# samson6460/tf2_YOLO

Measured on AMD Instinct MI355X. Metric: images/sec training YOLOv3 416x416 bs=32/GPU, higher is better.
Workload: dtype f32-storage/fp16x2-mfma

## Files before the change

### include/yolo_hip.h

```cpp
#ifndef YOLO_HIP_H_
#define YOLO_HIP_H_

#include <stddef.h>
#include <stdint.h>

#ifdef __cplusplus
extern "C" {
#endif

typedef enum yolo_status {
  YOLO_OK = 0,
  YOLO_ERR_INVALID_ARG = -1,
  YOLO_ERR_LAUNCH = -2,
  YOLO_ERR_WORKSPACE = -3
} yolo_status;

enum { YOLO_ACT_LINEAR = 0, YOLO_ACT_LEAKY = 1, YOLO_ACT_MISH = 2 };
enum { YOLO_HEAD_V3 = 3, YOLO_HEAD_V2 = 2, YOLO_HEAD_V1 = 1, YOLO_HEAD_V4 = 4 };
enum { YOLO_NMS_HARD = 1, YOLO_NMS_SOFT = 2, YOLO_NMS_DIOU = 3 };

const char* yolo_last_error(void);
int yolo_abi_version(void);
int yolo_device_available(void);
int yolo_mfma_probe(const void* operands_f16, float* sink, int workgroups, int iters, double* flops_host, void* stream);
// ... 9 lines not shown
typedef struct yolo_conv_desc {
  int N, H, W, Cin;
  int Cout, kh, kw;
  int Ho, Wo;
  int sh, sw;
  int pad_t, pad_l;
} yolo_conv_desc;

#define YOLO_BN_STAT_SLOTS 64
#define YOLO_BN_RED_SLOTS 512
#define YOLO_SPLIT_BATCH_UNITS 4

int yolo_conv2d_fwd(const yolo_conv_desc* d, const float* x, const float* w,
                    const float* bias, float* y, double* stats, void* stream);
int yolo_conv2d_fwd_absmax(const yolo_conv_desc* d, const float* x, const float* w, const float* bias,
                           float* y, double* stats, unsigned* absmax, void* stream);

int yolo_conv2d_dgrad(const yolo_conv_desc* d, const float* dy, const float* wT,
                      float* dx, int accumulate, void* stream);

int yolo_conv2d_wgrad(const yolo_conv_desc* d, const float* x, const float* dy,
                      float* dw, float* dbias, void* stream);

int yolo_conv2d_wgrad_bias(const float* dy, long long P, int Cout, float* dbias, void* stream);

int yolo_filter_transpose(const float* w, float* wT, int Cout, int taps, int Cin, void* stream);

size_t yolo_planes_bytes(long long rows, int C);
int yolo_split_planes(const float* x, long long rows, int C, void* planes, void* stream);
int yolo_split_planes_padded(const float* x, long long rows, int C_src, int C, void* planes, void* stream);

int yolo_split_planes_batch(const void* jobs, int njobs, long long total_blocks, void* stream);
int yolo_filter_transpose_batch(const void* jobs, int njobs, long long total_blocks, void* stream);

int yolo_conv2d_fwd_planes(const yolo_conv_desc* d, const void* x_planes, const void* w_planes,
                           const float* bias, float* y, double* stats, unsigned* absmax, void* stream);
int yolo_conv2d_dgrad_planes(const yolo_conv_desc* d, const void* dy_planes, const void* wT_planes,
                             float* dx, int accumulate, void* stream);
enum { YOLO_EPI_NONE = 0, YOLO_EPI_AFFINE = 1, YOLO_EPI_AFFINE_LEAKY = 2, YOLO_EPI_AFFINE_MISH = 3 };
int yolo_conv2d_fwd_planes_epi(const yolo_conv_desc* d, const void* x_planes, const void* w_planes, const float* bias,
                               int epilogue, const float* scale, const float* shift, const float* residual, float* y,
                               unsigned* absmax, void* stream);
int yolo_split_planes_absmax(const float* x, long long rows, int C, const unsigned* absmax, const float* extra_bound,
                             void* planes, float* out_bound, void* stream);
#define YOLO_INFER_BOUND_WORDS 4096
int yolo_conv_pred_bound(const float* w, int Cout, int kdim, const float* scale, const float* shift, const float* bias,
                         float* pred2, void* stream);
int yolo_conv2d_fwd_infer_unit(const yolo_conv_desc* d, const void* x_planes, const void* w_planes, const float* bias,
                               int epilogue, const float* scale, const float* shift, const float* residual, float* y,
                               unsigned* absmax, const float* pred2, const void* in_bound, int in_n,
                               const void* residual_bound, int residual_n, void* out_planes, unsigned* out_words,
                               float* out_bound, int* out_n_host, void* stream);
int yolo_fold_bound(const void* words, int n, float* out_bound, void* stream);
int yolo_absmax_words(const float* x, long long n, unsigned* words, int* n_words_host, void* stream);
int yolo_stem_filter_prep(const float* w, const float* bias, float* wt, void* stream);
int yolo_stem_fwd_infer_unit(const yolo_conv_desc* d, const float* x, const float* wt, int epilogue, const float* scale,
                             const float* shift, const float* pred2, const void* in_bound, int in_n, float* y,
                             void* out_planes, unsigned* out_words, int* out_n_host, void* stream);
int yolo_split_planes_concat(const float* const* srcs_host, const int* channels_host, const float* const* bounds_host,
                             int nsrc, long long rows, void* planes, float* dst32, float* out_bound, void* stream);
int yolo_split_planes_concat_ex(const float* const* srcs_host, const int* channels_host, const float* const* bounds_host,
                                const int* bound_words_host, const int* upsample_host, int H, int W, int nsrc,
                                long long rows, void* planes, float* dst32, float* out_bound, void* stream);
int yolo_conv2d_fwd_head_unit(const yolo_conv_desc* d, const void* x_planes, const void* w_planes, const float* bias,
                              int A, int C, int version, const float* anchors, float* t, float* y, void* stream);
int yolo_conv2d_wgrad_planes(const yolo_conv_desc* d, const void* x_planes, const void* dy_planes,
// ... 189 lines not shown
```

### tf2_yolo_amd/_lib.py

```python
import ctypes
import os
from ctypes import (POINTER, Structure, c_char_p, c_double, c_float, c_int, c_longlong,
                    c_size_t, c_void_p)

from . import tape as _tape

_HERE = os.path.dirname(os.path.abspath(__file__))
LIB_PATH = os.path.join(_HERE, "libyolo_hip.so")

ACT_LINEAR, ACT_LEAKY, ACT_MISH = 0, 1, 2
NMS_HARD, NMS_SOFT, NMS_DIOU = 1, 2, 3


class YoloHipError(RuntimeError):
    pass


class ConvDesc(Structure):
    _fields_ = [(n, c_int) for n in
                ("N", "H", "W", "Cin", "Cout", "kh", "kw", "Ho", "Wo", "sh", "sw", "pad_t", "pad_l")]


class LossCfg(Structure):
    _fields_ = [("version", c_int), ("N", c_int), ("gh", c_int), ("gw", c_int), ("A", c_int),
                ("C", c_int), ("anchors", c_float * 32), ("use_anchors", c_int),
                ("binary_weight", c_float), ("loss_weight", c_float * 4),
                ("ignore_thresh", c_float), ("use_focal_loss", c_int), ("focal_gamma", c_float),
                ("use_scale", c_int), ("wh_reg_weight", c_float), ("truth_thresh", c_float),
                ("label_smooth", c_float)]


_P = c_void_p
_LL = c_longlong
SIGNATURES = {
    "yolo_last_error": (c_char_p, []),
    "yolo_abi_version": (c_int, []),
    "yolo_device_available": (c_int, []),
    "yolo_set_option": (c_int, [c_int, c_int]),
    "yolo_mfma_probe": (c_int, [_P, _P, c_int, c_int, POINTER(c_double), _P]),
    "yolo_set_debug_buffer": (c_int, [_P, c_size_t]),
    "yolo_encode_labels": (c_int, [_P, _P, _P, c_int, c_double, c_double, c_int, c_int, c_int, _P, _P, _P]),
    "yolo_down2xlabel": (c_int, [_P, c_int, c_int, c_int, c_int, _P, _P, _P]),
    "yolo_conv_workspace_bytes": (c_size_t, []),
    "yolo_set_conv_workspace": (c_int, [_P, c_size_t, _P]),
    "yolo_conv2d_fwd": (c_int, [POINTER(ConvDesc), _P, _P, _P, _P, _P, _P]),
    "yolo_conv2d_dgrad": (c_int, [POINTER(ConvDesc), _P, _P, _P, c_int, _P]),
    "yolo_conv2d_wgrad": (c_int, [POINTER(ConvDesc), _P, _P, _P, _P, _P]),
    "yolo_conv2d_wgrad_bias": (c_int, [_P, _LL, c_int, _P, _P]),
    "yolo_filter_transpose": (c_int, [_P, _P, c_int, c_int, c_int, _P]),
    "yolo_planes_bytes": (c_size_t, [_LL, c_int]),
    "yolo_split_planes": (c_int, [_P, _LL, c_int, _P, _P]),
    "yolo_split_planes_padded": (c_int, [_P, _LL, c_int, c_int, _P, _P]),
    "yolo_split_planes_batch": (c_int, [_P, c_int, _LL, _P]),
    "yolo_filter_transpose_batch": (c_int, [_P, c_int, _LL, _P]),
    "yolo_conv2d_fwd_planes": (c_int, [POINTER(ConvDesc), _P, _P, _P, _P, _P, _P, _P]),
    "yolo_stem_bwd_scratch_bytes": (c_size_t, []),
    "yolo_stem_bn_bwd_wgrad": (c_int, [POINTER(ConvDesc), _P, _P, _P, _P, _P, _P, _P, c_int, _P, _P, _P, _P, _P, c_size_t, _P]),
    "yolo_conv2d_fwd_planes_epi": (c_int, [POINTER(ConvDesc), _P, _P, _P, c_int, _P, _P, _P, _P, _P, _P]),
    "yolo_split_planes_absmax": (c_int, [_P, _LL, c_int, _P, _P, _P, _P, _P]),
    "yolo_conv_pred_bound": (c_int, [_P, c_int, c_int, _P, _P, _P, _P, _P]),
    "yolo_conv2d_fwd_infer_unit": (c_int, [POINTER(ConvDesc), _P, _P, _P, c_int, _P, _P, _P, _P, _P, _P, _P, c_int, _P, c_int,
                                           _P, _P, _P, POINTER(c_int), _P]),
    "yolo_fold_bound": (c_int, [_P, c_int, _P, _P]),
    "yolo_absmax_words": (c_int, [_P, _LL, _P, POINTER(c_int), _P]),
    "yolo_stem_filter_prep": (c_int, [_P, _P, _P, _P]),
    "yolo_stem_fwd_infer_unit": (c_int, [POINTER(ConvDesc), _P, _P, c_int, _P, _P, _P, _P, c_int, _P, _P, _P, POINTER(c_int), _P]),
    "yolo_split_planes_concat": (c_int, [POINTER(c_void_p), POINTER(c_int), POINTER(c_void_p), c_int, _LL, _P, _P, _P, _P]),
    "yolo_split_planes_concat_ex": (c_int, [POINTER(c_void_p), POINTER(c_int), POINTER(c_void_p), POINTER(c_int), POINTER(c_int),
                                            c_int, c_int, c_int, _LL, _P, _P, _P, _P]),
    "yolo_conv2d_fwd_head_unit": (c_int, [POINTER(ConvDesc), _P, _P, _P, c_int, c_int, c_int, _P, _P, _P, _P]),
    "yolo_conv2d_fwd_absmax": (c_int, [POINTER(ConvDesc), _P, _P, _P, _P, _P, _P, _P]),
    "yolo_conv2d_dgrad_planes": (c_int, [POINTER(ConvDesc), _P, _P, _P, c_int, _P]),
    "yolo_conv2d_wgrad_planes": (c_int, [POINTER(ConvDesc), _P, _P, _P, _P]),
    "yolo_wgrad_workspace_bytes": (c_size_t, []),
    "yolo_set_wgrad_workspace": (c_int, [_P, c_size_t]),
    "yolo_bn_stats": (c_int, [_P, _LL, c_int, _P, _P]),
    "yolo_bn_finalize": (c_int, [_P, _LL, c_int, _P, _P, c_float, c_float, c_int, _P, _P, _P, _P, _P, _P, _P]),
    "yolo_bn_fold_inference": (c_int, [c_int, _P, _P, _P, _P, c_float, _P, _P, _P]),
    "yolo_bn_act_fwd": (c_int, [_P, _LL, c_int, _P, _P, c_int, _P, _P, _P]),
    "yolo_bn_act_bwd_reduce": (c_int, [_P, _P, _LL, c_int, _P, _P, _P, _P, c_int, _P, _P]),
    "yolo_bn_act_bwd_apply": (c_int, [_P, _P, _LL, c_int, _P, _P, _P, _P, _P, c_int, _P, _P, _P, _P, _P]),
    "yolo_bn_act_fwd_planes": (c_int, [_P, _LL, c_int, _P, _P, c_int, _P, _P, _P, _P, _P, _P, _P]),
    "yolo_bn_act_fwd_res_planes": (c_int, [_P, _LL, c_int, _P, _P, c_int, _P, _P, _P, _P, _P, _P]),
    "yolo_bn_act_bwd_apply_planes": (c_int, [_P, _P, _LL, c_int, _P, _P, _P, _P, _P, c_int, _P, _P, _P, _P, _P, _P,
                                             _P]),
    "yolo_bn_infer_bound": (c_int, [c_int, _P, _P, _P, _P, _P]),
    "yolo_bn_finalize_bound": (c_int, [_P, _LL, c_int, _P, _P, c_float, c_float, c_int, _P, _P, _P, _P, _P, _P, _P,
# ... 116 lines not shown
```

### tf2_yolo_amd/csrc/conv.hip

```cpp
#include "conv_args.hpp"
#include <cstdlib>
#include <type_traits>

namespace yolo {

template <int BM, int BN, int WGM, int WGN, bool FLAT>
__global__ __launch_bounds__(256) void gather_conv_kernel(const GatherConvArgs a) {
  constexpr int BK = 32;
  constexpr int LD = BK + 4;
  constexpr int TM = BM / WGM / 32;
  constexpr int TN = BN / WGN / 32;
  constexpr int AR = BM / 32;
  constexpr int BR = BN / 32;
  static_assert(WGM * WGN == 4, "4 waves per block");
  static_assert(TM >= 1 && TN >= 1, "wave tile");

  extern __shared__ __attribute__((aligned(16))) float smem[];
  constexpr int BUF = (BM + BN) * LD;

  const int tid = threadIdx.x;
  const int lane = tid & 63;
  const int wave = tid >> 6;
  const int wm = wave / WGN, wn = wave % WGN;

// ... 982 lines not shown
  a.dst = t;
  fill_fwd_args(d, a);
  YOLO_REQUIRE(gather_planes_supported(a), "conv_fwd_head_unit: needs Cin %% 16 == 0 and Cout >= 32");
  if ((version == YOLO_HEAD_V3 || version == YOLO_HEAD_V4) && anchors != nullptr) {
    a.head_y = y;
    a.head_anchors = anchors;
    a.head_A = A;
    a.head_C = C;
    if (conv_small_head_supported(a)) {
      int nwg = 0;
      return launch_conv_small(a, as_stream(stream), &nwg);
    }
    a.head_y = nullptr;
  }
  if (int rc = launch_gather_planes(a, as_stream(stream))) return rc;
  return yolo_head_act_fwd(t, (long long)d->N * d->Ho * d->Wo, A, C, version, anchors, y, stream);
}

extern "C" size_t yolo_planes_bytes(long long rows, int C) {
  if (rows <= 0 || C <= 0 || (C % 16) != 0) return 0;
  return (size_t)planes_bytes(rows, C);
}

extern "C" int yolo_split_planes_batch(const void* jobs, int njobs, long long total_blocks, void* stream) {
  YOLO_REQUIRE(jobs, "split_planes_batch: null job table");
  return launch_split_planes_batch(jobs, njobs, total_blocks, as_stream(stream));
}

extern "C" int yolo_filter_transpose_batch(const void* jobs, int njobs, long long total_blocks, void* stream) {
  YOLO_REQUIRE(jobs, "filter_transpose_batch: null job table");
  return launch_filter_transpose_batch(jobs, njobs, total_blocks, as_stream(stream));
}

extern "C" int yolo_split_planes(const float* x, long long rows, int C, void* planes, void* stream) {
  YOLO_REQUIRE(x && planes, "split_planes: null pointer");
  return launch_split_planes(x, rows, C, planes, as_stream(stream));
}

extern "C" int yolo_split_planes_padded(const float* x, long long rows, int C_src, int C, void* planes, void* stream) {
  YOLO_REQUIRE(x && planes, "split_planes_padded: null pointer");
  return launch_split_planes_padded(x, rows, C_src, C, planes, as_stream(stream));
}

struct BnRedArgs {
  const float* y;
  const float* scale;
  const float* shift;
  const float* mean;
  const float* invstd;
  int act;
  float* part;
  int cap;
  unsigned* aux;
  int nslots;
};
static void set_bnred(GatherConvArgs& a, const BnRedArgs* b) {
  if (b == nullptr) return;
  a.bwd_y = b->y; a.bwd_scale = b->scale; a.bwd_shift = b->shift; a.bwd_mean = b->mean; a.bwd_invstd = b->invstd;
  a.bwd_act = b->act; a.bwd_part = b->part; a.bwd_cap = b->cap; a.bwd_aux = b->aux;
}

static int dgrad_impl(const yolo_conv_desc* d, const float* dy, const float* wT, float* dx, int accumulate,
                      void* stream, bool planes, BnRedArgs* bnred = nullptr) {
  if (int rc = validate_desc(d)) return rc;
  YOLO_REQUIRE(dy && wT && dx, "conv_dgrad: null pointer");
  const bool flat = (d->Cout % 32) != 0;
// ... 214 lines not shown
```

### tf2_yolo_amd/csrc/conv_args.hpp

```cpp
#pragma once
#include "common.hpp"

namespace yolo {

constexpr int MAX_TAPS = 49;

struct Tap {
  int oy, ox, woff;
};

struct ClassGeom {
  long long M;
  int Hg, Wg, ooy, oox, tap0, ntaps;
};

struct GatherConvArgs {
  const float* src;
  const float* wgt;
  const float* bias;
  float* dst;
  double* stats;
  unsigned* absmax;
  long long M;
  int N, Hs, Ws, Cs;
// ... 62 lines not shown

struct WgradArgs {
  const float* src;
  const float* dy;
  float* dw;
  long long M;
  int N, Hs, Ws, Cs;
  int Hg, Wg;
  int sy, sx;
  int Cout, ldw;
  int ntaps;
  int kw, pad_t, pad_l;
  int tiles_co, tiles_j;
  int nblocks;
  long long chunk;
  unsigned src_bytes, dy_bytes;
  int zero_blk_src, zero_blk_dy;
  float* slabs;
  int splits;
};

int launch_gather_split(GatherConvArgs& a, hipStream_t st);
bool gather_split_supported(const GatherConvArgs& a);
long long planes_bytes(long long rows, int C);
int launch_split_planes(const float* x, long long rows, int C, void* planes, hipStream_t st);
int launch_split_planes_absmax(const float* x, long long rows, int C, const unsigned* absmax, const float* extra_bound, int extra_n,
                               void* planes, float* out_bound, hipStream_t st);
int launch_split_planes_concat(const float* const* xs, const int* Cs, const float* const* bounds, int nsrc, long long rows,
                               void* planes, float* dst32, float* out_bound, hipStream_t st,
                               const int* bound_words = nullptr, const int* upsample = nullptr, int H = 0, int W = 0);
int launch_split_planes_padded(const float* x, long long rows, int Csrc, int C, void* planes, hipStream_t st);
int launch_split_planes_batch(const void* jobs, int njobs, long long total_blocks, hipStream_t st);
int launch_filter_transpose_batch(const void* jobs, int njobs, long long total_blocks, hipStream_t st);
int launch_gather_planes(GatherConvArgs& a, hipStream_t st);
bool conv_small_supported(const GatherConvArgs& a);
bool conv_small_head_supported(const GatherConvArgs& a);
int launch_conv_small(GatherConvArgs& a, hipStream_t st, int* nwg);
bool gather_planes_supported(const GatherConvArgs& a);
int conv_split_parts(const GatherConvArgs& a, long long nb, int bm, int min_cb, int idle_div);
int launch_split_reduce(GatherConvArgs& a, int bm, hipStream_t st);
float* conv_split_slabs();
int launch_conv_win(GatherConvArgs& a, int variant, hipStream_t st);
bool conv_win_supported(const GatherConvArgs& a);
enum { OPT_CONV_WIN = 0, OPT_STAMPS = 1, OPT_CONV_SK = 2, OPT_DBG = 3, OPT_TILE_ORDER = 4, OPT_CONV_PATCH = 5, OPT_WGRAD_WIN = 6, OPT_NMS_WALK = 7, OPT_EXP = 8, OPT_COUNT = 16 };
int set_conv_workspace(void* p, size_t bytes, hipStream_t st);
extern void* g_dbg_buf;
extern size_t g_dbg_bytes;
extern int g_opt[OPT_COUNT];
void init_options();
int launch_wgrad_planes(WgradArgs& a, hipStream_t st);
bool wgrad_planes_supported(const WgradArgs& a);
int launch_wgrad_win(WgradArgs& a, hipStream_t st);
bool wgrad_win_supported(const WgradArgs& a);
constexpr size_t WGRAD_WS_COLSUM_BYTES = 1 << 20;
void* wgrad_workspace(size_t* bytes);
bool stem_fwd_supported(const yolo_conv_desc* d);
struct StemEpiArgs {
  const float* scale;
  const float* shift;
  int act;
  void* planes;
  const float* pred;
  const unsigned* in_words;
  int in_n;
  unsigned* out_words;
};
// ... 16 lines not shown
```

### tf2_yolo_amd/csrc/conv_planes.hip

```cpp
#include "planes_epilogue.hpp"
#include <algorithm>
#include <cstdlib>
#include <type_traits>

namespace yolo {

__global__ __launch_bounds__(256) void planes_amax_kernel(const float* __restrict__ x, long long n4,
                                                         unsigned* __restrict__ header) {
  float m = 0.f;
  for (long long i = (long long)blockIdx.x * 256 + threadIdx.x; i < n4; i += (long long)gridDim.x * 256) {
    const f32x4 v = reinterpret_cast<const f32x4*>(x)[i];
    m = fmaxf(fmaxf(m, fmaxf(fabsf(v[0]), fabsf(v[1]))), fmaxf(fabsf(v[2]), fabsf(v[3])));
  }
#pragma unroll
  for (int o = 32; o > 0; o >>= 1) m = fmaxf(m, __shfl_xor(m, o, 64));
  __shared__ float wmax[4];
  if ((threadIdx.x & 63) == 0) wmax[threadIdx.x >> 6] = m;
  __syncthreads();
  if (threadIdx.x == 0) {
    m = fmaxf(fmaxf(wmax[0], wmax[1]), fmaxf(wmax[2], wmax[3]));
    if (__builtin_bit_cast(unsigned, m) > *reinterpret_cast<volatile unsigned*>(header))
      atomicMax(header, __builtin_bit_cast(unsigned, m));
  }
}
// ... 603 lines not shown
                               void* planes, float* dst32, float* out_bound, hipStream_t st, const int* bound_words,
                               const int* upsample, int H, int W) {
  ConcatSrcs cs{};
  int C = 0;
  cs.H = H;
  cs.W = W;
  for (int i = 0; i < nsrc; ++i) {
    cs.x[i] = xs[i];
    cs.bound[i] = bounds[i];
    cs.bound_n[i] = bound_words != nullptr ? bound_words[i] : 1;
    cs.up[i] = upsample != nullptr ? upsample[i] : 0;
    cs.C[i] = Cs[i];
    C += Cs[i];
    cs.g_end[i] = C >> 3;
  }
  cs.n = nsrc;
  const long long rows_padded = ((rows + 15) / 16 + 1) * 16;
  const int G = C >> 3;
  const long long blocks = ((rows_padded + 16 * SPLIT_BLOCKS_PER_WG - 1) / (16 * SPLIT_BLOCKS_PER_WG)) * ((G + 15) >> 4);
  if (blocks <= 0 || blocks > 0x7fffffffLL) {
    set_error("split_planes_concat: bad grid %lld", blocks);
    return YOLO_ERR_INVALID_ARG;
  }
  hipLaunchKernelGGL(split_planes_concat_kernel, dim3((unsigned)blocks), dim3(256), 0, st, cs, rows, C,
                     reinterpret_cast<unsigned char*>(planes), rows_padded, dst32, out_bound);
  return check_launch("split_planes_concat_kernel");
}

struct BatchJob {
  const void* src;
  void* dst;
  long long a, b, c, first_block;
};
__device__ __forceinline__ int find_job(const BatchJob* jobs, int njobs, long long block) {
  int lo = 0, hi = njobs - 1;
  while (lo < hi) {
    const int mid = (lo + hi + 1) >> 1;
    if (jobs[mid].first_block <= block) lo = mid;
    else hi = mid - 1;
  }
  return lo;
}

__global__ void planes_header_clear_batch_kernel(const BatchJob* __restrict__ jobs, int njobs) {
  const int i = blockIdx.x * blockDim.x + threadIdx.x;
  if (i >= njobs) return;
  unsigned* header = reinterpret_cast<unsigned*>(reinterpret_cast<unsigned char*>(jobs[i].dst) +
                                                 planes_body_bytes(jobs[i].a, (int)jobs[i].b));
  header[0] = 0u;
}
constexpr int BATCH_UNITS = YOLO_SPLIT_BATCH_UNITS;
struct BatchPos {
  long long row0;
  int g;
  bool live;
};
__device__ __forceinline__ BatchPos batch_pos(const BatchJob& j) {
  const int G = (int)j.b >> 3;
  const int gbn = (G + 15) >> 4;
  const long long lb = (long long)blockIdx.x - j.first_block;
  const long long rb = lb / gbn;
  const int gb = (int)(lb - rb * gbn);
  BatchPos p;
  p.g = gb * 16 + (threadIdx.x >> 4);
  p.row0 = rb * (16 * BATCH_UNITS) + (threadIdx.x & 15);
  p.live = p.g < G;
  return p;
// ... 62 lines not shown
  for (int u = 0; u < BATCH_UNITS; ++u) {
    const long long row = p.row0 + 16 * u;
    if (row >= rows_padded) continue;
    const Planes8 s8 = split8(v[u][0], v[u][1], sc);
    unsigned char* o = out + planes_unit_offset(row, p.g, C);
    *reinterpret_cast<u32x4*>(o) = s8.h;
    *reinterpret_cast<u32x4*>(o + 512) = s8.l;
  }
}

__global__ __launch_bounds__(256) void filter_transpose_batch_kernel(const BatchJob* __restrict__ jobs, int njobs) {
  __shared__ float tile[32][33];
  const BatchJob j = jobs[find_job(jobs, njobs, blockIdx.x)];
  const float* w = reinterpret_cast<const float*>(j.src);
  float* wT = reinterpret_cast<float*>(j.dst);
  const int Cout = (int)j.a, taps = (int)j.b, Cin = (int)j.c;
  const int bx = (Cin + 31) / 32, by = (Cout + 31) / 32;
  const int lb = (int)((long long)blockIdx.x - j.first_block);
  const int t = lb / (bx * by);
  const int rem = lb - t * (bx * by);
  const int co0 = (rem / bx) * 32, ci0 = (rem % bx) * 32;
  const int tx = threadIdx.x & 31, ty = threadIdx.x >> 5;
  for (int r = ty; r < 32; r += 8) {
    const int co = co0 + r, ci = ci0 + tx;
    tile[r][tx] = (co < Cout && ci < Cin) ? w[((long long)co * taps + t) * Cin + ci] : 0.f;
  }
  __syncthreads();
  for (int r = ty; r < 32; r += 8) {
    const int ci = ci0 + r, co = co0 + tx;
    if (ci < Cin && co < Cout) wT[((long long)ci * taps + t) * Cout + co] = tile[tx][r];
  }
}

int launch_split_planes_batch(const void* jobs, int njobs, long long total_blocks, hipStream_t st) {
  if (njobs <= 0 || total_blocks <= 0 || total_blocks > 0x7fffffffLL) {
    set_error("split_planes_batch: bad job table");
    return YOLO_ERR_INVALID_ARG;
  }
  const BatchJob* jb = reinterpret_cast<const BatchJob*>(jobs);
  hipLaunchKernelGGL(planes_header_clear_batch_kernel, dim3((njobs + 255) / 256), dim3(256), 0, st, jb, njobs);
  hipLaunchKernelGGL(planes_amax_batch_kernel, dim3((unsigned)total_blocks), dim3(256), 0, st, jb, njobs);
  hipLaunchKernelGGL(split_planes_batch_kernel, dim3((unsigned)total_blocks), dim3(256), 0, st, jb, njobs);
  return check_launch("split_planes_batch_kernel");
}

int launch_filter_transpose_batch(const void* jobs, int njobs, long long total_blocks, hipStream_t st) {
  if (njobs <= 0 || total_blocks <= 0 || total_blocks > 0x7fffffffLL) {
    set_error("filter_transpose_batch: bad job table");
    return YOLO_ERR_INVALID_ARG;
  }
  hipLaunchKernelGGL(filter_transpose_batch_kernel, dim3((unsigned)total_blocks), dim3(256), 0, st,
                     reinterpret_cast<const BatchJob*>(jobs), njobs);
  return check_launch("filter_transpose_batch_kernel");
}

int launch_split_planes_padded(const float* x, long long rows, int Csrc, int C, void* planes, hipStream_t st) {
  if (C % 16 != 0 || rows <= 0 || Csrc <= 0 || Csrc > C || C - Csrc >= 16) {
    set_error("split_planes_padded: need 0 < Csrc <= C < Csrc + 16, C %% 16 == 0, rows > 0");
    return YOLO_ERR_INVALID_ARG;
  }
  const long long rows_padded = ((rows + 15) / 16 + 1) * 16;
  const long long blocks = (rows_padded * (C / 8) + 255) / 256;
  if (blocks > 0x7fffffffLL) {
    set_error("split_planes_padded: tensor too large");
    return YOLO_ERR_INVALID_ARG;
  }
// ... 57 lines not shown
```

### tf2_yolo_amd/engine.py

```python
import math

import contextlib
import os

import numpy as np
import torch

from . import ops
from . import tape
from ._lib import ACT_LEAKY, ACT_LINEAR, ACT_MISH, YoloHipError

AUX_WORDS = 112

ACT_NAMES = {ACT_LINEAR: "linear", ACT_LEAKY: "leaky", ACT_MISH: "mish"}


class ParamSpec:
    __slots__ = ("name", "shape", "offset", "size", "init", "trainable")

    def __init__(self, name, shape, offset, init, trainable):
        self.name, self.shape, self.offset = name, tuple(shape), offset
        self.size = int(np.prod(shape))
        self.init, self.trainable = init, trainable

# ... 328 lines not shown
                has_planes_src = any(c.kind in ("conv", "head") and c.src.tid == u.out.tid and c.planes_fwd for c in cs)
                u.a_needed = ((not cs) or (u.out.tid in out_tids) or u.cout % 16 != 0 or not has_planes_src
                              or any(not reads_planes_only(c) for c in cs))
        self._pool_fuse = os.environ.get("YOLO_POOL_FUSE", "1") != "0"
        for u in self.units:
            u.pool_fuse = None
        if self._pool_fuse:
            for u in self.units:
                if u.kind != "conv" or not u.bn or u.residual is not None or u.out.tid in out_tids:
                    continue
                cs = consumers.get(u.out.tid, [])
                if len(cs) != 1 or cs[0].kind != "maxpool":
                    continue
                p = cs[0]
                if (p.k == 2 and p.stride == 2 and u.out.h % 2 == 0 and u.out.w % 2 == 0 and p.out.h * 2 == u.out.h
                        and p.out.w * 2 == u.out.w and u.cout % 8 == 0 and p.padding in ("same", "valid")):
                    pcs = consumers.get(p.out.tid, [])
                    p.f32_needed = (p.out.tid in out_tids) or (not pcs) or p.out.c % 16 != 0 or any(
                        not (c.kind in ("conv", "head") and c.src.tid == p.out.tid and c.planes_fwd and c.planes_wgrad
                             and getattr(c, "residual", None) is not p.out) for c in pcs)
                    u.pool_fuse = p
        self._concat_planes = os.environ.get("YOLO_CONCAT_PLANES", "1") != "0"
        self._bound_alias = {}
        for u in self.units:
            if u.kind in ("upsample", "maxpool", "space_to_depth"):
                self._bound_alias[u.out.tid] = self._bound_alias.get(u.src.tid, u.src.tid)
            elif u.kind == "concat":
                cs = consumers.get(u.out.tid, [])
                u.f32_needed = (u.out.tid in out_tids) or (not cs) or any(
                    not (c.kind in ("conv", "head") and c.src.tid == u.out.tid and c.planes_fwd and c.planes_wgrad
                         and getattr(c, "residual", None) is not u.out) for c in cs)
        self._wp_valid = False
        self._wTp_valid = False
        self._jobs_wp = self._jobs_wTp = self._jobs_wT = None
        off = 0
        for u in self.units:
            u.aux_off = off
            off += AUX_WORDS
            if u.kind == "conv" and u.bn:
                off += (u.cout + 7) // 8 * 8
        ntb = max(len(self.tensors), 1) + 1
        self._aux = torch.zeros(max(off, 1) + ntb, device=self.device, dtype=torch.int32)
        self._tbound = self._aux[max(off, 1):].view(torch.float32)
        self._twords = None
        self._tword_n = {}
        self._pred = torch.zeros(2 * max(len(self.units), 1), device=self.device, dtype=torch.float32)
        for i, u in enumerate(self.units):
            u.pred_off = 2 * i
        self._infer_onepass = os.environ.get("YOLO_INFER_ONEPASS", "1") != "0"
        self._infer_small_fuse = os.environ.get("YOLO_INFER_SMALL_FUSE", "1") != "0"
        self._up_producer = {}
        for u in self.units:
            u.concat_reads_through = False
            if u.kind == "upsample" and self._n_consumers.get(u.out.tid, 0) == 1 and u.out.tid not in out_tids:
                cs = consumers.get(u.out.tid, [])
                if (len(cs) == 1 and cs[0].kind == "concat" and u.out.h == 2 * u.src.h and u.out.w == 2 * u.src.w
                        and u.out.c == u.src.c):
                    self._up_producer[u.out.tid] = u
        self._xplanes_infer = {}

    def _declare_params(self):
        wT = 0
        f32 = 0
        f64 = 0
        for u in self.units:
            if u.kind == "conv":
                cin = u.src.c
# ... 158 lines not shown
            for u in self.units:
                if u.kind == "head" and u.cpad:
                    nb = ops.planes_bytes(N * u.out.h * u.out.w, u.cpad)
                elif u.kind in ("conv", "head") and (u.planes_dgrad or u.planes_wgrad):
                    nb = ops.planes_bytes(N * u.out.h * u.out.w, u.cout if u.kind == "conv" else u.out.c)
                else:
                    continue
                self._dyp_own[u.name] = torch.empty(nb, device=dev, dtype=torch.uint8)
        self._xp_valid = set()

    def _tb_row(self, tid):
        if self._twords is None:
            self._twords = torch.zeros((max(len(self.tensors), 1) + 1) * ops.INFER_BOUND_WORDS, device=self.device,
                                       dtype=torch.int32)
        return self._twords[tid * ops.INFER_BOUND_WORDS:(tid + 1) * ops.INFER_BOUND_WORDS]

    def _tb_float(self, tid):
        n = self._tword_n.pop(tid, 0)
        if n:
            ops.fold_bound(self._tb_row(tid)[:n], self._tbound[tid:tid + 1])
        return self._tbound[tid:tid + 1]

    def _tb_words(self, tid):
        n = self._tword_n.get(tid, 0)
        return self._tb_row(tid)[:n] if n else self._tbound[tid:tid + 1]

    def _xp(self, t):
        buf = self._xplanes[t.tid]
        if t.tid not in self._xp_valid:
            ops.split_planes(self.act[t.tid], self.batch * t.h * t.w, t.c, out=buf)
            self._xp_valid.add(t.tid)
        return buf

    def _refresh_wplanes(self):
        if self._wp_valid or self._wplanes is None:
            return
        if self._jobs_wp is None:
            self._jobs_wp = ops.BatchJobs("split", self.device)
            for u in self.units:
                if u.kind in ("conv", "head") and u.planes_fwd:
                    cout = u.cout if u.kind == "conv" else u.out.c
                    k = u.k if u.kind == "conv" else 1
                    self._jobs_wp.add_split(self.params.view(u.p_kernel.name),
                                            self._wplanes[u.wp_off:u.wp_off + u.wp_bytes], cout, k * k * u.src.c)
        self._jobs_wp.run()
        self._wp_valid = True

    def _refresh_wTplanes(self):
        if self._wTp_valid or self._wplanes is None:
            return
        self._refresh_wplanes()
        if self._jobs_wTp is None:
            self._jobs_wTp = ops.BatchJobs("split", self.device)
            for u in self.units:
                if u.kind == "head" and u.cpad:
                    self._jobs_wTp.add_split(u.wT_pad, self._wplanes[u.wTp_pad_off:u.wTp_pad_off + u.wTp_pad_bytes],
                                             u.src.c, u.cpad)
                elif u.kind in ("conv", "head") and u.planes_dgrad:
                    cout = u.cout if u.kind == "conv" else u.out.c
                    k = u.k if u.kind == "conv" else 1
                    n = cout * k * k * u.src.c
                    donor = self._wplanes[u.wp_off:u.wp_off + u.wp_bytes] if u.planes_fwd else None
                    self._jobs_wTp.add_split(self._wT[u.wT_off:u.wT_off + n],
                                             self._wplanes[u.wTp_off:u.wTp_off + u.wTp_bytes], u.src.c, k * k * cout,
                                             bound_from=donor)
        self._jobs_wTp.run()
        self._wTp_valid = True

    def _conv_fwd(self, u, xin, w, bias, out, stats=None):
        amax = self._aux[u.aux_off + AUX_WORDS:u.aux_off + AUX_WORDS + u.cout] if (stats is not None and self._tight_bound(u)) else None
        if u.planes_fwd:
            return ops.conv2d_fwd_planes(u.desc, self._xp(u.src), self._wplanes[u.wp_off:u.wp_off + u.wp_bytes], bias,
                                         out=out, stats=stats, absmax=amax)
        return ops.conv2d_fwd(u.desc, xin, w, bias, out=out, stats=stats, absmax=amax)

    def _tight_bound(self, u):
        m = self._bn_tight
        return m == 1 or (m == 2 and u.k != 1)

    def _bn_bufs(self, u):
        c = u.cout
        b = self._bn_f32[u.bn_f32_off:u.bn_f32_off + 4 * c]
        ns = ops.BN_STAT_SLOTS * 2 * c
# ... 26 lines not shown
            if ev is not None:
                torch.cuda.current_stream().wait_event(ev)
        self._wp_event = self._wT_event = None

    def mark_params_changed(self):
        self.before_param_write()
        self._infer_graphs = {}
        self._wT_valid = False
        self._wp_valid = False
        self._wTp_valid = False
        self._infer_scale_valid = False

    def forward(self, x, training=False, stop_after=None):
        if x.dtype != torch.float32 or not x.is_cuda:
            raise YoloHipError("forward expects a float32 CUDA tensor")
        x = x.contiguous()
        N = x.shape[0]
        if tuple(x.shape[1:]) != (self.input.h, self.input.w, self.input.c):
            raise YoloHipError(f"input shape {tuple(x.shape[1:])} != model input "
                               f"{(self.input.h, self.input.w, self.input.c)}")
        self.allocate(N)
        self.training = training
        self.act[self.input.tid] = x
        self._xp_valid = set()
        self._tbound_set = set()
        self._tword_n = {}
        if training and self._overlap_wgrad and self._prep_beside and not (self._wp_valid and self._wT_valid and self._wTp_valid):
            if self._wgrad_stream is None:
                self._wgrad_stream = ops.concurrent_stream("wgrad", device=self.device)
            side = self._wgrad_stream
            tape.wait_stream(side, torch.cuda.current_stream())
            with torch.cuda.stream(side):
                self._refresh_wplanes()
                self._wp_event = tape.record_event(side)
                self._refresh_wT()
                self._refresh_wTplanes()
                self._wT_event = tape.record_event(side)
        else:
            self._refresh_wplanes()
        ops.zero_bytes(self._aux)
        if training:
            ops.zero_bytes(self._bn_f64[:self._bn_stats_total])
            self._infer_scale_valid = False
            self._infer_graphs = {}
        P = self.params
        prev_name = None
        for u in self.units:
            if stop_after is not None and prev_name == stop_after:
                self.training = False
                return None
            prev_name = getattr(u, "name", None)
            if self._wp_event is not None and u.kind in ("conv", "head") and u.planes_fwd:
                tape.wait_event(torch.cuda.current_stream(), self._wp_event)
                self._wp_event = None
            if u.kind == "conv":
                xin = self.act[u.src.tid]
                w = P.view(u.p_kernel.name)
                bias = P.view(u.p_bias.name) if u.p_bias is not None else None
                if u.bn:
                    scale, shift, smean, sinv, stats, _ = self._bn_bufs(u)
                    gamma, beta = P.view(u.p_gamma.name), P.view(u.p_beta.name)
                    if training:
                        self._conv_fwd(u, xin, w, None, u.y, stats)
                        ops.bn_finalize(stats, u.y.numel() // u.cout, u.cout, gamma, beta,
                                        self.state.view(u.s_mean.name), self.state.view(u.s_var.name),
                                        scale, shift, smean, sinv, unbiased=self.unbiased_moving_var,
                                        bound=self._aux[u.aux_off:u.aux_off + 1],
                                        absmax=(self._aux[u.aux_off + AUX_WORDS:u.aux_off + AUX_WORDS + u.cout]
                                                if self._tight_bound(u) else None), mean_offset=bias)
                    elif self._fuse_infer and self._fused_infer_unit(u, bias, gamma, beta, scale, shift):
# ... 169 lines not shown
                self._tword_n[u.out.tid] = nw
            self._tbound_set.add(u.out.tid)
            if own_planes:
                self._xp_valid.add(u.out.tid)
            return True
        if not own_planes:
            return False
        ops.conv2d_fwd_planes_epi(u.desc, self._xp(u.src), self._wplanes[u.wp_off:u.wp_off + u.wp_bytes], bias, epi, scale,
                                  shift, residual=res, out=u.a, absmax=amax)
        ops.split_planes_absmax(u.a, self.batch * u.out.h * u.out.w, u.cout, amax, pl,
                                extra_bound=self._tb_float(u.residual.tid) if u.residual is not None else None,
                                out_bound=tb[u.out.tid:u.out.tid + 1])
        self._tbound_set.add(u.out.tid)
        self._xp_valid.add(u.out.tid)
        return True

    def _takes_grad_slice(self, u):
        if u.kind != "conv" or not u.bn or u.residual is not None or u.cout % 8 != 0:
            return False
        need_pl = u.planes_wgrad or u.planes_dgrad
        if self._stem_fused and not need_pl and not self._needs_grad[u.src.tid] and ops.stem_bn_bwd_supported(u.desc):
            return False
        return True

    def _add_grad(self, grads, t, buf):
        if not self._needs_grad[t.tid]:
            return
        cur = grads.get(t.tid)
        if cur is None:
            grads[t.tid] = buf
        else:
            ops.axpy(cur, buf)

    def _refresh_wT(self):
        if self._wT_valid:
            return
        if self._jobs_wT is None:
            self._jobs_wT = ops.BatchJobs("transpose", self.device)
            for u in self.units:
                if u.kind == "head" and u.cpad:
                    self._jobs_wT.add_transpose(u.w_pad, u.wT_pad, u.cpad, 1, u.src.c)
                elif u.kind in ("conv", "head"):
                    cout = u.cout if u.kind == "conv" else u.out.c
                    taps = u.k * u.k if u.kind == "conv" else 1
                    n = cout * taps * u.src.c
                    self._jobs_wT.add_transpose(self.params.view(u.p_kernel.name), self._wT[u.wT_off:u.wT_off + n],
                                                cout, taps, u.src.c)
        for u in self.units:
            if u.kind == "head" and u.cpad:
                tape.torch_op(lambda u=u: u.w_pad[:u.out.c * u.src.c].copy_(self.params.view(u.p_kernel.name).reshape(-1)))
        self._jobs_wT.run()
        self._wT_valid = True

    def _gview(self, spec):
        return self.grads[spec.offset:spec.offset + spec.size]

    def backward(self, douts):
        if not self.training:
            raise YoloHipError("backward() requires a preceding forward(training=True)")
        if self.backward_begin_hook is not None:
            tape.host_call(self.backward_begin_hook)
        if self._wT_event is not None:
            tape.wait_event(torch.cuda.current_stream(), self._wT_event)
            self._wT_event = None
        self._refresh_wT()
        self._refresh_wTplanes()
        for u in self.units:
            if getattr(u, "bnred", None) is not None:
                u.bnred_done = False
        grads = {}
        for t, g in zip(self.outputs, douts):
            grads[t.tid] = g
        N = self.batch
        for u in reversed(self.units):
            dout = grads.pop(u.out.tid, None)
            if dout is None:
                continue
            if isinstance(dout, ops.ChannelSlice) and not self._takes_grad_slice(u):
                dout = dout.dense((N, u.out.h, u.out.w, u.out.c))
            if u.kind == "conv":
                xin = self.act[u.src.tid]
                if u.bn:
# ... 229 lines not shown
```

### tf2_yolo_amd/ops.py

```python
import ctypes
from ctypes import byref, c_void_p

import torch

from . import _lib
from . import tape as _tape
from ._lib import ConvDesc, LossCfg, YoloHipError, check

BN_EPS = 1e-3
BN_MOMENTUM = 0.99
BN_STAT_SLOTS = 64
BN_RED_SLOTS = 512
SPLIT_BATCH_UNITS = 4


class KernelTimer:

    def __init__(self):
        self.pending = []

    def bracket(self, name, flops, launches, fn, layer=None):
        s, e = torch.cuda.Event(enable_timing=True), torch.cuda.Event(enable_timing=True)
        s.record()
        fn()
# ... 293 lines not shown

def split_planes_padded(x, rows, c_src, out=None):
    _chk_f32(x)
    c = (c_src + 15) // 16 * 16
    if x.numel() != rows * c_src:
        raise YoloHipError("split_planes_padded: tensor size does not match rows x C_src")
    n = planes_bytes(rows, c)
    if out is None:
        out = torch.empty(n, device=x.device, dtype=torch.uint8)
    elif out.numel() < n or out.dtype != torch.uint8:
        raise YoloHipError("split_planes_padded: output buffer too small")
    check(_lib.load().yolo_split_planes_padded(_p(x), int(rows), int(c_src), int(c), _p(out), _stream()),
          "yolo_split_planes_padded")
    return out


class BatchJobs:

    def __init__(self, kind, device):
        self.kind, self.device = kind, device
        self.rows, self.blocks, self.table = [], 0, None

    def add_split(self, src, dst, rows, c, bound_from=None):
        nb = -(-((rows + 15) // 16 + 1) // SPLIT_BATCH_UNITS) * -(-c // 128)
        donor = 0 if bound_from is None else bound_from.data_ptr() + bound_from.numel() - 256
        self.rows.append([src.data_ptr(), dst.data_ptr(), rows, c, donor, self.blocks])
        self.blocks += nb

    def add_transpose(self, src, dst, cout, taps, cin):
        nb = -(-cin // 32) * -(-cout // 32) * taps
        self.rows.append([src.data_ptr(), dst.data_ptr(), cout, taps, cin, self.blocks])
        self.blocks += nb

    def run(self):
        if not self.rows:
            return
        if self.table is None:
            self.table = torch.tensor(self.rows, dtype=torch.int64).to(self.device)
        fn = _lib.load().yolo_split_planes_batch if self.kind == "split" else _lib.load().yolo_filter_transpose_batch
        check(fn(_p(self.table), len(self.rows), self.blocks, _stream()), "yolo_%s_batch" % self.kind)


def conv2d_fwd_planes(d, xp, wp, bias=None, out=None, stats=None, absmax=None):
    _chk_f32(bias)
    if out is None:
        out = torch.empty((d.N, d.Ho, d.Wo, d.Cout), device=xp.device, dtype=torch.float32)
    if xp.numel() < planes_bytes(d.N * d.H * d.W, d.Cin) or wp.numel() < planes_bytes(d.Cout, d.kh * d.kw * d.Cin):
        raise YoloHipError("conv2d_fwd_planes: planes buffers do not match the descriptor")
    if out.numel() != d.N * d.Ho * d.Wo * d.Cout:
        raise YoloHipError("conv2d_fwd_planes: output size does not match the descriptor")
    if stats is not None and stats.numel() != BN_STAT_SLOTS * 2 * d.Cout:
        raise YoloHipError("conv2d_fwd_planes: stats must hold BN_STAT_SLOTS x 2 x Cout doubles")
    def run():
        check(_lib.load().yolo_conv2d_fwd_planes(byref(d), _p(xp), _p(wp), _p(bias), _p(out), _p(stats), _p(absmax),
                                                 _stream()), "yolo_conv2d_fwd_planes")
    if TIMER is not None:
        TIMER.bracket(_planes_variant(d.Cout, _win_key(d, d.H, d.W, d.Cin), d.kh * d.kw == 1), _conv_flops(d), 1, run,
                      _layer_key(d, "fwd"))
    else:
        run()
    return out


EPI_NONE, EPI_AFFINE, EPI_AFFINE_LEAKY, EPI_AFFINE_MISH = 0, 1, 2, 3


def conv2d_fwd_planes_epi(d, xp, wp, bias, epilogue, scale, shift, residual=None, out=None, absmax=None):
    _chk_f32(bias, scale, shift, residual)
    if out is None:
        out = torch.empty((d.N, d.Ho, d.Wo, d.Cout), device=xp.device, dtype=torch.float32)
    if xp.numel() < planes_bytes(d.N * d.H * d.W, d.Cin) or wp.numel() < planes_bytes(d.Cout, d.kh * d.kw * d.Cin):
        raise YoloHipError("conv2d_fwd_planes_epi: planes buffers do not match the descriptor")
# ... 780 lines not shown
```

Before: 1084.

## Fuse filter plane splitting and transpose into batched amax and planes kernels

Adds a fused weight-preparation path. One batched kernel computes each filter's absmax bound. A second kernel then writes both the forward fp16 hi/lo weight planes and the transposed dgrad planes directly from the fp32 filters, using an LDS tile for the transpose. This replaces the previous sequence of split, transpose, split-transposed and head-padding copies, cutting per-step launches and the extra HBM round-trips through the fp32 transposed buffer. It is enabled by default when every unit's shape passes the alignment checks. It adds an atomic bound-reduction pass and a more complex indexing scheme that must match the existing planes layout.

```diff
diff --git a/include/yolo_hip.h b/include/yolo_hip.h
--- a/include/yolo_hip.h
+++ b/include/yolo_hip.h
@@ -65,6 +65,8 @@
 
 int yolo_split_planes_batch(const void* jobs, int njobs, long long total_blocks, void* stream);
 int yolo_filter_transpose_batch(const void* jobs, int njobs, long long total_blocks, void* stream);
+int yolo_filter_amax_batch(const void* jobs, int njobs, long long total_blocks, void* stream);
+int yolo_filter_planes_batch(const void* jobs, int njobs, long long total_blocks, void* stream);
 
 int yolo_conv2d_fwd_planes(const yolo_conv_desc* d, const void* x_planes, const void* w_planes,
                            const float* bias, float* y, double* stats, unsigned* absmax, void* stream);
diff --git a/tf2_yolo_amd/_lib.py b/tf2_yolo_amd/_lib.py
--- a/tf2_yolo_amd/_lib.py
+++ b/tf2_yolo_amd/_lib.py
@@ -53,6 +53,8 @@
     "yolo_split_planes_padded": (c_int, [_P, _LL, c_int, c_int, _P, _P]),
     "yolo_split_planes_batch": (c_int, [_P, c_int, _LL, _P]),
     "yolo_filter_transpose_batch": (c_int, [_P, c_int, _LL, _P]),
+    "yolo_filter_amax_batch": (c_int, [_P, c_int, _LL, _P]),
+    "yolo_filter_planes_batch": (c_int, [_P, c_int, _LL, _P]),
     "yolo_conv2d_fwd_planes": (c_int, [POINTER(ConvDesc), _P, _P, _P, _P, _P, _P, _P]),
     "yolo_stem_bwd_scratch_bytes": (c_size_t, []),
     "yolo_stem_bn_bwd_wgrad": (c_int, [POINTER(ConvDesc), _P, _P, _P, _P, _P, _P, _P, c_int, _P, _P, _P, _P, _P, c_size_t, _P]),
diff --git a/tf2_yolo_amd/csrc/conv.hip b/tf2_yolo_amd/csrc/conv.hip
--- a/tf2_yolo_amd/csrc/conv.hip
+++ b/tf2_yolo_amd/csrc/conv.hip
@@ -1038,6 +1038,16 @@
   return launch_filter_transpose_batch(jobs, njobs, total_blocks, as_stream(stream));
 }
 
+extern "C" int yolo_filter_amax_batch(const void* jobs, int njobs, long long total_blocks, void* stream) {
+  YOLO_REQUIRE(jobs, "filter_amax_batch: null job table");
+  return launch_filter_amax_batch(jobs, njobs, total_blocks, as_stream(stream));
+}
+
+extern "C" int yolo_filter_planes_batch(const void* jobs, int njobs, long long total_blocks, void* stream) {
+  YOLO_REQUIRE(jobs, "filter_planes_batch: null job table");
+  return launch_filter_planes_batch(jobs, njobs, total_blocks, as_stream(stream));
+}
+
 extern "C" int yolo_split_planes(const float* x, long long rows, int C, void* planes, void* stream) {
   YOLO_REQUIRE(x && planes, "split_planes: null pointer");
   return launch_split_planes(x, rows, C, planes, as_stream(stream));
diff --git a/tf2_yolo_amd/csrc/conv_args.hpp b/tf2_yolo_amd/csrc/conv_args.hpp
--- a/tf2_yolo_amd/csrc/conv_args.hpp
+++ b/tf2_yolo_amd/csrc/conv_args.hpp
@@ -118,6 +118,8 @@
 int launch_split_planes_padded(const float* x, long long rows, int Csrc, int C, void* planes, hipStream_t st);
 int launch_split_planes_batch(const void* jobs, int njobs, long long total_blocks, hipStream_t st);
 int launch_filter_transpose_batch(const void* jobs, int njobs, long long total_blocks, hipStream_t st);
+int launch_filter_amax_batch(const void* jobs, int njobs, long long total_blocks, hipStream_t st);
+int launch_filter_planes_batch(const void* jobs, int njobs, long long total_blocks, hipStream_t st);
 int launch_gather_planes(GatherConvArgs& a, hipStream_t st);
 bool conv_small_supported(const GatherConvArgs& a);
 bool conv_small_head_supported(const GatherConvArgs& a);
diff --git a/tf2_yolo_amd/csrc/conv_planes.hip b/tf2_yolo_amd/csrc/conv_planes.hip
--- a/tf2_yolo_amd/csrc/conv_planes.hip
+++ b/tf2_yolo_amd/csrc/conv_planes.hip
@@ -659,7 +659,8 @@
   void* dst;
   long long a, b, c, first_block;
 };
-__device__ __forceinline__ int find_job(const BatchJob* jobs, int njobs, long long block) {
+template <typename Job>
+__device__ __forceinline__ int find_job(const Job* jobs, int njobs, long long block) {
   int lo = 0, hi = njobs - 1;
   while (lo < hi) {
     const int mid = (lo + hi + 1) >> 1;
@@ -788,6 +789,168 @@
   }
 }
 
+struct FusedJob {
+  const void* src;
+  void* dst_w;
+  void* dst_wT;
+  long long Cout, taps, Cin;
+  long long Cout_pad;
+  unsigned* bound;
+  long long first_block;
+  long long reserved;
+};
+constexpr int FP_CO = 16 * BATCH_UNITS;
+constexpr int FP_CI = 128;
+constexpr int FP_PITCH = FP_CI + 4;
+struct FusedPos {
+  int co0, t, ci0;
+};
+__device__ __forceinline__ FusedPos fused_pos(const FusedJob& j) {
+  const long long nbi = (j.Cin + 15) / 16 + (j.dst_wT != nullptr ? 1 : 0);
+  const int nit = (int)((nbi + FP_CI / 16 - 1) / (FP_CI / 16));
+  const long long lb = (long long)blockIdx.x - j.first_block;
+  const long long ct_t = lb / nit;
+  FusedPos p;
+  p.ci0 = (int)(lb - ct_t * nit) * FP_CI;
+  p.t = (int)(ct_t % j.taps);
+  p.co0 = (int)(ct_t / j.taps) * FP_CO;
+  return p;
+}
+__device__ __forceinline__ void fused_load(const FusedJob& j, const FusedPos& p, f32x4 (&v)[BATCH_UNITS][2]) {
+  const float* w = reinterpret_cast<const float*>(j.src);
+  const int r = threadIdx.x & 15, ci = p.ci0 + (threadIdx.x >> 4) * 8;
+#pragma unroll
+  for (int u = 0; u < BATCH_UNITS; ++u) {
+    const int co = p.co0 + 16 * u + r;
+    v[u][0] = v[u][1] = f32x4{0.f, 0.f, 0.f, 0.f};
+    if (co < j.Cout && ci < j.Cin) {
+      const float* q = w + ((long long)co * j.taps + p.t) * j.Cin + ci;
+      v[u][0] = *reinterpret_cast<const f32x4*>(q);
+      v[u][1] = *reinterpret_cast<const f32x4*>(q + 4);
+    }
+  }
+}
+__global__ void filter_bound_clear_batch_kernel(const FusedJob* __restrict__ jobs, int njobs) {
+  const int i = blockIdx.x * blockDim.x + threadIdx.x;
+  if (i < njobs) *jobs[i].bound = 0u;
+}
+__global__ __launch_bounds__(256) void filter_amax_batch_kernel(const FusedJob* __restrict__ jobs, int njobs) {
+  const FusedJob j = jobs[find_job(jobs, njobs, blockIdx.x)];
+  const FusedPos p = fused_pos(j);
+  if (p.co0 >= j.Cout || p.ci0 >= j.Cin) return;
+  f32x4 v[BATCH_UNITS][2];
+  fused_load(j, p, v);
+  float m = 0.f;
+#pragma unroll
+  for (int u = 0; u < BATCH_UNITS; ++u)
+#pragma unroll
+    for (int h = 0; h < 2; ++h)
+      m = fmaxf(m, fmaxf(fmaxf(fabsf(v[u][h][0]), fabsf(v[u][h][1])), fmaxf(fabsf(v[u][h][2]), fabsf(v[u][h][3]))));
+#pragma unroll
+  for (int o = 32; o > 0; o >>= 1) m = fmaxf(m, __shfl_xor(m, o, 64));
+  if ((threadIdx.x & 63) == 0 && m > 0.f) {
+    if (__builtin_bit_cast(unsigned, m) > *reinterpret_cast<volatile unsigned*>(j.bound))
+      atomicMax(j.bound, __builtin_bit_cast(unsigned, m));
+  }
+}
+__global__ __launch_bounds__(256) void filter_planes_batch_kernel(const FusedJob* __restrict__ jobs, int njobs) {
+  __shared__ unsigned tile[FP_CO * FP_PITCH];
+  const FusedJob j = jobs[find_job(jobs, njobs, blockIdx.x)];
+  const int Cout = (int)j.Cout, taps = (int)j.taps, Cin = (int)j.Cin, Cout_pad = (int)j.Cout_pad;
+  unsigned char* ow = reinterpret_cast<unsigned char*>(j.dst_w);
+  unsigned char* oT = reinterpret_cast<unsigned char*>(j.dst_wT);
+  const int Cw = taps * Cin, CT = taps * Cout_pad;
+  const unsigned bound = *j.bound;
+  const float sc = planes_scale_from_bound(bound);
+  if ((long long)blockIdx.x == j.first_block && threadIdx.x == 0) {
+    if (ow != nullptr) {
+      unsigned* header = reinterpret_cast<unsigned*>(ow + planes_body_bytes(Cout, Cw));
+      header[0] = bound;
+      reinterpret_cast<float*>(header)[1] = sc;
+      reinterpret_cast<float*>(header)[2] = 1.f / sc;
+    }
+    if (oT != nullptr) {
+      unsigned* header = reinterpret_cast<unsigned*>(oT + planes_body_bytes(Cin, CT));
+      header[0] = bound;
+      reinterpret_cast<float*>(header)[1] = sc;
+      reinterpret_cast<float*>(header)[2] = 1.f / sc;
+    }
+  }
+  const FusedPos p = fused_pos(j);
+  const bool data = p.co0 < Cout && p.ci0 < Cin;
+  const int r = threadIdx.x & 15, gg = threadIdx.x >> 4;
+  const int ci = p.ci0 + gg * 8;
+  f32x4 v[BATCH_UNITS][2];
+  fused_load(j, p, v);
+  const int rows_padded_w = ((Cout + 15) / 16 + 1) * 16;
+#pragma unroll
+  for (int u = 0; u < BATCH_UNITS; ++u) {
+    const int co = p.co0 + 16 * u + r;
+    const Planes8 s8 = split8(v[u][0], v[u][1], sc);
+    if (ow != nullptr && ci < Cin && co < rows_padded_w) {
+      unsigned char* o = ow + planes_unit_offset(co, (p.t * Cin + ci) >> 3, Cw);
+      *reinterpret_cast<u32x4*>(o) = s8.h;
+      *reinterpret_cast<u32x4*>(o + 512) = s8.l;
+    }
+    if (oT != nullptr && data) {
+      unsigned* q = tile + (16 * u + r) * FP_PITCH + gg * 8;
+      u32x4 a, b;
+#pragma unroll
+      for (int i = 0; i < 2; ++i) {
+        a[2 * i] = (s8.h[i] & 0xffffu) | (s8.l[i] << 16);
+        a[2 * i + 1] = (s8.h[i] >> 16) | (s8.l[i] & 0xffff0000u);
+        b[2 * i] = (s8.h[2 + i] & 0xffffu) | (s8.l[2 + i] << 16);
+        b[2 * i + 1] = (s8.h[2 + i] >> 16) | (s8.l[2 + i] & 0xffff0000u);
+      }
+      *reinterpret_cast<u32x4*>(q) = a;
+      *reinterpret_cast<u32x4*>(q + 4) = b;
+    }
+  }
+  if (oT == nullptr) return;
+  if (data) __syncthreads();
+  const int cl = threadIdx.x & (FP_CI - 1), q8 = threadIdx.x >> 7;
+  const int rowT = p.ci0 + cl;
+  if (rowT >= ((Cin + 15) / 16 + 1) * 16) return;
+#pragma unroll
+  for (int u = 0; u < BATCH_UNITS; ++u) {
+    const int cb = p.co0 + 16 * u;
+    if (cb >= Cout_pad) break;
+    unsigned e[8];
+#pragma unroll
+    for (int k = 0; k < 8; ++k) e[k] = data ? tile[(16 * u + 8 * q8 + k) * FP_PITCH + cl] : 0u;
+    u32x4 h, l;
+#pragma unroll
+    for (int i = 0; i < 4; ++i) {
+      h[i] = (e[2 * i] & 0xffffu) | (e[2 * i + 1] << 16);
+      l[i] = (e[2 * i] >> 16) | (e[2 * i + 1] & 0xffff0000u);
+    }
+    unsigned char* o = oT + planes_unit_offset(rowT, ((p.t * Cout_pad + cb) >> 3) + q8, CT);
+    *reinterpret_cast<u32x4*>(o) = h;
+    *reinterpret_cast<u32x4*>(o + 512) = l;
+  }
+}
+
+int launch_filter_amax_batch(const void* jobs, int njobs, long long total_blocks, hipStream_t st) {
+  if (njobs <= 0 || total_blocks <= 0 || total_blocks > 0x7fffffffLL) {
+    set_error("filter_amax_batch: bad job table");
+    return YOLO_ERR_INVALID_ARG;
+  }
+  const FusedJob* jb = reinterpret_cast<const FusedJob*>(jobs);
+  hipLaunchKernelGGL(filter_bound_clear_batch_kernel, dim3((njobs + 255) / 256), dim3(256), 0, st, jb, njobs);
+  hipLaunchKernelGGL(filter_amax_batch_kernel, dim3((unsigned)total_blocks), dim3(256), 0, st, jb, njobs);
+  return check_launch("filter_amax_batch_kernel");
+}
+
+int launch_filter_planes_batch(const void* jobs, int njobs, long long total_blocks, hipStream_t st) {
+  if (njobs <= 0 || total_blocks <= 0 || total_blocks > 0x7fffffffLL) {
+    set_error("filter_planes_batch: bad job table");
+    return YOLO_ERR_INVALID_ARG;
+  }
+  hipLaunchKernelGGL(filter_planes_batch_kernel, dim3((unsigned)total_blocks), dim3(256), 0, st,
+                     reinterpret_cast<const FusedJob*>(jobs), njobs);
+  return check_launch("filter_planes_batch_kernel");
+}
+
 int launch_split_planes_batch(const void* jobs, int njobs, long long total_blocks, hipStream_t st) {
   if (njobs <= 0 || total_blocks <= 0 || total_blocks > 0x7fffffffLL) {
     set_error("split_planes_batch: bad job table");
diff --git a/tf2_yolo_amd/engine.py b/tf2_yolo_amd/engine.py
--- a/tf2_yolo_amd/engine.py
+++ b/tf2_yolo_amd/engine.py
@@ -384,7 +384,9 @@
                          and getattr(c, "residual", None) is not u.out) for c in cs)
         self._wp_valid = False
         self._wTp_valid = False
-        self._jobs_wp = self._jobs_wTp = self._jobs_wT = None
+        self._jobs_wp = self._jobs_wTp = self._jobs_wT = self._jobs_fused = None
+        self._prep_fused = (os.environ.get("YOLO_PREP_FUSED", "1") != "0" and self._wplanes is not None
+                            and all(ops.BatchJobs.fused_ok(*self._fused_shape(u)) for u in self._fused_units()))
         off = 0
         for u in self.units:
             u.aux_off = off
@@ -609,9 +611,36 @@
             self._xp_valid.add(t.tid)
         return buf
 
+    def _fused_units(self):
+        return [u for u in self.units if u.kind in ("conv", "head") and (u.planes_fwd or u.planes_dgrad or u.cpad)]
+
+    def _fused_shape(self, u):
+        cout = u.cout if u.kind == "conv" else u.out.c
+        k = u.k if u.kind == "conv" else 1
+        return cout, k * k, u.src.c, (u.cpad or cout), u.planes_fwd, bool(u.planes_dgrad or u.cpad)
+
+    def _refresh_planes_fused(self):
+        if self._jobs_fused is None:
+            units = self._fused_units()
+            self._wbound = torch.zeros(max(len(units), 1), device=self.device, dtype=torch.int32)
+            self._jobs_fused = ops.BatchJobs("fused", self.device)
+            for i, u in enumerate(units):
+                cout, taps, cin, cout_pad, has_w, has_wT = self._fused_shape(u)
+                if u.cpad:
+                    wT_dst = self._wplanes[u.wTp_pad_off:u.wTp_pad_off + u.wTp_pad_bytes]
+                else:
+                    wT_dst = self._wplanes[u.wTp_off:u.wTp_off + u.wTp_bytes] if has_wT else None
+                self._jobs_fused.add_fused(self.params.view(u.p_kernel.name),
+                                           self._wplanes[u.wp_off:u.wp_off + u.wp_bytes] if has_w else None, wT_dst,
+                                           cout, taps, cin, cout_pad, self._wbound[i:i + 1])
+        self._jobs_fused.run()
+        self._wp_valid = self._wTp_valid = True
+
     def _refresh_wplanes(self):
         if self._wp_valid or self._wplanes is None:
             return
+        if self._prep_fused:
+            return self._refresh_planes_fused()
         if self._jobs_wp is None:
             self._jobs_wp = ops.BatchJobs("split", self.device)
             for u in self.units:
@@ -626,6 +655,8 @@
     def _refresh_wTplanes(self):
         if self._wTp_valid or self._wplanes is None:
             return
+        if self._prep_fused:
+            return self._refresh_planes_fused()
         self._refresh_wplanes()
         if self._jobs_wTp is None:
             self._jobs_wTp = ops.BatchJobs("split", self.device)
@@ -718,10 +749,16 @@
             tape.wait_stream(side, torch.cuda.current_stream())
             with torch.cuda.stream(side):
                 self._refresh_wplanes()
-                self._wp_event = tape.record_event(side)
-                self._refresh_wT()
-                self._refresh_wTplanes()
-                self._wT_event = tape.record_event(side)
+                if self._prep_fused:
+                    self._wp_event = self._wT_event = tape.record_event(side)
+                    self._refresh_wT()
+                    if self._jobs_wT.rows:
+                        self._wT_event = tape.record_event(side)
+                else:
+                    self._wp_event = tape.record_event(side)
+                    self._refresh_wT()
+                    self._refresh_wTplanes()
+                    self._wT_event = tape.record_event(side)
         else:
             self._refresh_wplanes()
         ops.zero_bytes(self._aux)
@@ -957,6 +994,9 @@
         else:
             ops.axpy(cur, buf)
 
+    def _reads_wT(self, u):
+        return self._needs_grad[u.src.tid] and not u.planes_dgrad and not (u.kind == "head" and u.cpad)
+
     def _refresh_wT(self):
         if self._wT_valid:
             return
@@ -964,15 +1004,16 @@
             self._jobs_wT = ops.BatchJobs("transpose", self.device)
             for u in self.units:
                 if u.kind == "head" and u.cpad:
-                    self._jobs_wT.add_transpose(u.w_pad, u.wT_pad, u.cpad, 1, u.src.c)
-                elif u.kind in ("conv", "head"):
+                    if not self._prep_fused:
+                        self._jobs_wT.add_transpose(u.w_pad, u.wT_pad, u.cpad, 1, u.src.c)
+                elif u.kind in ("conv", "head") and (not self._prep_fused or self._reads_wT(u)):
                     cout = u.cout if u.kind == "conv" else u.out.c
                     taps = u.k * u.k if u.kind == "conv" else 1
                     n = cout * taps * u.src.c
                     self._jobs_wT.add_transpose(self.params.view(u.p_kernel.name), self._wT[u.wT_off:u.wT_off + n],
                                                 cout, taps, u.src.c)
         for u in self.units:
-            if u.kind == "head" and u.cpad:
+            if u.kind == "head" and u.cpad and not self._prep_fused:
                 tape.torch_op(lambda u=u: u.w_pad[:u.out.c * u.src.c].copy_(self.params.view(u.p_kernel.name).reshape(-1)))
         self._jobs_wT.run()
         self._wT_valid = True
diff --git a/tf2_yolo_amd/ops.py b/tf2_yolo_amd/ops.py
--- a/tf2_yolo_amd/ops.py
+++ b/tf2_yolo_amd/ops.py
@@ -349,12 +349,38 @@
         self.rows.append([src.data_ptr(), dst.data_ptr(), cout, taps, cin, self.blocks])
         self.blocks += nb
 
-    def run(self):
+    @staticmethod
+    def fused_ok(cout, taps, cin, cout_pad, has_w, has_wT):
+        return ((has_w or has_wT) and cin % 8 == 0 and cout_pad in (cout, (cout + 15) // 16 * 16)
+                and (not has_w or (taps * cin) % 16 == 0) and (not has_wT or cout_pad % 16 == 0))
+
+    def add_fused(self, src, dst_w, dst_wT, cout, taps, cin, cout_pad, bound):
+        if not self.fused_ok(cout, taps, cin, cout_pad, dst_w is not None, dst_wT is not None):
+            raise YoloHipError("filter_planes_batch: unsupported shape %s" % ((cout, taps, cin, cout_pad),))
+        if src.numel() != cout * taps * cin or bound.numel() != 1 or bound.element_size() != 4:
+            raise YoloHipError("filter_planes_batch: filter / bound word size does not match the shape")
+        if ((dst_w is not None and dst_w.numel() < planes_bytes(cout, taps * cin))
+                or (dst_wT is not None and dst_wT.numel() < planes_bytes(cin, taps * cout_pad))):
+            raise YoloHipError("filter_planes_batch: planes buffer too small")
+        nbo = (cout + 15) // 16 + 1 if dst_w is not None else cout_pad // 16
+        nbi = (cin + 15) // 16 + (1 if dst_wT is not None else 0)
+        nb = -(-nbo // SPLIT_BATCH_UNITS) * taps * -(-nbi // 8)
+        self.rows.append([src.data_ptr(), 0 if dst_w is None else dst_w.data_ptr(), 0 if dst_wT is None else dst_wT.data_ptr(),
+                          cout, taps, cin, cout_pad, bound.data_ptr(), self.blocks, 0])
+        self.blocks += nb
+
+    def run(self, amax=True):
         if not self.rows:
             return
         if self.table is None:
             self.table = torch.tensor(self.rows, dtype=torch.int64).to(self.device)
-        fn = _lib.load().yolo_split_planes_batch if self.kind == "split" else _lib.load().yolo_filter_transpose_batch
+        lib = _lib.load()
+        if self.kind == "fused":
+            if amax:
+                check(lib.yolo_filter_amax_batch(_p(self.table), len(self.rows), self.blocks, _stream()), "yolo_filter_amax_batch")
+            check(lib.yolo_filter_planes_batch(_p(self.table), len(self.rows), self.blocks, _stream()), "yolo_filter_planes_batch")
+            return
+        fn = lib.yolo_split_planes_batch if self.kind == "split" else lib.yolo_filter_transpose_batch
         check(fn(_p(self.table), len(self.rows), self.blocks, _stream()), "yolo_%s_batch" % self.kind)
 
 
```

Result: no change. 1083 (median of 3 runs) (-0.0%).
